# bleyerj/dolfinx_materials

Hardware: AMD Instinct MI355X
Metric: M quadrature-point updates/s (stress+tangent, fp64) (higher is better)
Workload: dtype f64; 1 GPU; cfg2: J2 von-Mises plasticity, linear isotropic hardening, small strain, 1e+07 Gauss points per GPU, stress + 6x6 consistent tangent, load/unload history increments 2-4; points_per_gpu=10000000, law=j2_linear, layout=AoS (N,6)/(N,36) boundary arrays in HBM, SoA resident state, placement=every array where its first allocation put it, settle_launches_before_warmup=560

## Files before the change

### dolfinx_materials_amd/csrc/dxmat.hip

```cpp
#include <hip/hip_runtime.h>

#include <algorithm>
#include <atomic>
#include <chrono>
#include <cmath>
#include <condition_variable>
#include <deque>
#include <map>
#include <mutex>
#include <thread>
#include <cstdarg>
#include <cstdio>
#include <cstdlib>
#include <cstring>
#include <string>
#include <vector>

#include "../../include/dxmat.h"
#include "dxm_common.hpp"
#include "fefp.hpp"
#include "gradient.hpp"
#include "small_strain.hpp"
#include "ramberg_osgood.hpp"
#include "param_fields.hpp"
#include "hyperelastic.hpp"
#include "hosford.hpp"
#include "orthotropic.hpp"
#include "host_side.hpp"

using namespace dxm;
static_assert(TL_FULL == DXM_TANGENT_FULL && TL_SYM == DXM_TANGENT_SYM && TL_COEF == DXM_TANGENT_COEF && TL_PACK4 == DXM_TANGENT_PACK4, "kernel and ABI layout ids");

static thread_local std::string g_last_error;

static int fail(int code, const char* fmt, ...) {
  char buf[512];
  va_list ap;
  va_start(ap, fmt);
  vsnprintf(buf, sizeof(buf), fmt, ap);
  va_end(ap);
  g_last_error = buf;
  return code;
}

#define HIP_TRY(expr)                                                                      \
  do {                                                                                     \
    hipError_t _e = (expr);                                                                \
    if (_e != hipSuccess) {                                                                \
      (void)hipGetLastError();                                                             \
      return fail(-2, "%s failed: %s (%s:%d)", #expr, hipGetErrorString(_e), __FILE__, __LINE__); \
    }                                                                                      \
  } while (0)

struct DeviceGuard {
  int prev = -1;
  bool ok = true;
  explicit DeviceGuard(int device) {
    if (hipGetDevice(&prev) != hipSuccess) prev = -1;
    if (prev != device) ok = (hipSetDevice(device) == hipSuccess);
  }
  ~DeviceGuard() {
    int cur = -1;
    if (prev >= 0 && hipGetDevice(&cur) == hipSuccess && cur != prev) (void)hipSetDevice(prev);
  }
};
#define DEVICE_GUARD(m)                                                        \
  DeviceGuard _guard((m)->device);                                             \
  if (!_guard.ok) return fail(-2, "hipSetDevice(%d) failed", (m)->device)

#ifdef DXM_CUSTOM_HARDENING
constexpr bool kCustomBuild = true;
#define DXM_STOCK_ONLY(entry) nullptr
#else
constexpr bool kCustomBuild = false;
#define DXM_STOCK_ONLY(entry) entry
#endif

struct dxm_material;

struct LaunchArgs {
  dxm_material* m;
  int grid;
  hipStream_t st;
  int64_t off, cnt;
  const double* grad;
  double* flux;
  double* ct;
  int stats_off;
  const MeshSource* fused;
  int tl;
};

constexpr unsigned L_FULL = 1u << TL_FULL, L_SYM = 1u << TL_SYM, L_COEF = 1u << TL_COEF, L_PACK4 = 1u << TL_PACK4;
constexpr unsigned L_ALL = L_FULL | L_SYM | L_COEF | L_PACK4;

struct LawDesc {
  int id;
  int n_grad, n_flux;
  int n_params, n_params_custom;
  int n_isv_fields;
  int n_fields;
  int isv_dim[DXM_MAX_STATE_FIELDS];
  const char* isv_name[DXM_MAX_STATE_FIELDS];
  int isv_slot[DXM_MAX_STATE_FIELDS];
  int n_slots;
  unsigned unit_fields;
  int alg_bytes;
  const char* kernel;
  const char* field_kernel;
  const char* no_fields;
  int (*build)(const double* p, LawParams& q);
  const char* stock_only;
  const void* (*residency_kernel)();
  int blocks_per_cu;
  unsigned set_layouts;
  const char* set_refusal;
  unsigned launch_layouts;
  const char* launch_refusal;
  const char* no_fused;
  const char* no_frame;
  const char* frame_kernel[2];
  void (*launch)(const LaunchArgs& a);
};

static int elastic_constants(const double* p, LawParams& q) {
  const double E = p[0], nu = p[1];
  if (!(E > 0.0) || !(nu > -1.0 && nu < 0.5)) return fail(-1, "invalid elastic constants E=%g nu=%g", E, nu);
  q.lambda = E * nu / (1 + nu) / (1 - 2 * nu);
  q.mu = E / 2 / (1 + nu);
  q.kappa = q.lambda + 2.0 * q.mu / 3.0;
  q.sig0 = 1.0;
  return 0;
}

static void yield_tolerance(LawParams& q) { q.tol = q.rtol * fmax(fabs(q.sig0), 2e-8 * q.mu); }

static int build_elastic(const double* p, LawParams& q) {
  if (int rc = elastic_constants(p, q)) return rc;
// ... 103 lines not shown
static void launch_hosford(const LaunchArgs& a);
static void launch_orthotropic(const LaunchArgs& a);

[[maybe_unused]] static const void* const kKernelOrder[5] = {
    (const void*)small_strain_kernel<LAW_ELASTIC, TL_FULL>, (const void*)small_strain_kernel<LAW_J2_LINEAR, TL_FULL>,
    (const void*)small_strain_kernel<LAW_J2_VOCE, TL_FULL>, (const void*)fefp_kernel<0, 0>, (const void*)fefp_kernel<1, 0>};


constexpr const char* kNoFrame = "this law is isotropic: a material frame changes nothing in its update, and accepting one would hide a "
                                 "mistake of the caller (frames are read by DXM_LAW_ORTHOTROPIC_ELASTIC)";

constexpr void state_field(LawDesc& d, int f, const char* name, int dim, int slot) {
  d.isv_name[f] = name; d.isv_dim[f] = dim; d.isv_slot[f] = slot;
}

constexpr LawDesc small_strain_law(int id, int n_params, int alg_bytes, const char* kernel, bool coef, void (*launch)(const LaunchArgs&)) {
  LawDesc d{};
  d.id = id;
  d.n_grad = d.n_flux = 6;
  d.n_params = d.n_params_custom = n_params;
  d.alg_bytes = alg_bytes;
  d.kernel = kernel;
  d.set_layouts = d.launch_layouts = coef ? L_ALL : L_FULL | L_SYM;
  d.no_frame = kNoFrame;
  d.launch = launch;
  return d;
}

constexpr void j2_state(LawDesc& d) {
  d.n_isv_fields = d.n_fields = 2;
  state_field(d, 0, "p", 1, 0);
  state_field(d, 1, "epsp", 6, 1);
  d.n_slots = SS_NSLOTS;
}

constexpr LawDesc law_elastic() {
  LawDesc d = small_strain_law(DXM_LAW_ELASTIC_ISO, 2, 384, "small_strain_kernel<0", false, launch_small_strain<LAW_ELASTIC>);
  d.build = build_elastic;
  d.residency_kernel = []() -> const void* { return (const void*)small_strain_kernel<LAW_ELASTIC, TL_FULL>; };
  d.blocks_per_cu = 32;
  d.set_refusal = d.launch_refusal = "the elastic tangent is the constant lambda 1x1 + 2 mu I: there are no per-point coefficients";
  d.no_fields = "the elastic tangent is a constant the host path never downloads";
  return d;
}

constexpr LawDesc law_j2_linear() {
  LawDesc d = small_strain_law(DXM_LAW_J2_LINEAR, 4, 496, "small_strain_kernel<1", true, launch_small_strain<LAW_J2_LINEAR>);
  j2_state(d);
  d.build = build_linear_hardening;
  d.residency_kernel = []() -> const void* { return (const void*)small_strain_kernel<LAW_J2_LINEAR, TL_FULL>; };
  d.blocks_per_cu = 32;
  d.field_kernel = "small_strain_field_kernel<1";
  return d;
}

constexpr LawDesc law_j2_voce() {
  LawDesc d = small_strain_law(DXM_LAW_J2_VOCE, 5, 496, "small_strain_kernel<2", true, launch_small_strain<LAW_J2_VOCE>);
  j2_state(d);
  d.n_params_custom = 9;
  d.build = build_voce_hardening;
  d.residency_kernel = []() -> const void* { return (const void*)small_strain_kernel<LAW_J2_VOCE, TL_FULL>; };
  d.blocks_per_cu = 256;
  d.field_kernel = "small_strain_field_kernel<2";
  return d;
}

// ... 135 lines not shown
static int tangent_size(const dxm_material* m);

static int isv_total(const LawDesc& d) {
  int t = 0;
  for (int f = 0; f < d.n_isv_fields; ++f) t += d.isv_dim[f];
  return t;
}

using dxm_host::HostPool;
using dxm_host::expand_coef_tangent;
using dxm_host::expand_pack4_tangent;
using dxm_host::expand_fefp_tangent;
using dxm_host::fill_const_tangent;
using dxm_host::CtRoute;
using dxm_host::Route;
static_assert(dxm_host::THIRD == SS_THIRD && dxm_host::FEFP_RECORD == FEFP_REC, "host rebuilds and kernels share these constants");

constexpr int DXM_MAX_CHUNKS = dxm_host::MAX_CHUNKS;
constexpr int DXM_RING = dxm_host::RING;

struct dxm_material {
  int law = 0;
  int device = 0;
  int64_t n = 0;
  int64_t ld = 0;
  LawParams prm{};
  std::vector<double> raw_params;
  int maxit = 25;
  double rtol = 1e-14;
  double* state[2] = {nullptr, nullptr};
  double* state_base = nullptr;
  size_t s1_skew = 0;
  bool s1_alias = false;
  BlockStats* d_stats = nullptr;
  BlockStats* h_stats = nullptr;
  int stats_capacity = 0;
  int last_grid = 0;
  hipStream_t pipe_stream = nullptr;
  hipStream_t down_stream2 = nullptr;
  hipEvent_t last_event = nullptr;
  bool last_event_recorded = false;
  bool launched = false;
  hipStream_t own_stream = nullptr;
  uint64_t epoch = 0;
  int parity = 0;
  bool opt_pipeline = true;
  bool opt_split_streams = true;
  int opt_packed_transfer = 2;
  bool opt_fused_gradient = true;
  bool opt_staged_gradient = true;
  bool opt_verbose = false;
  dxm_host::UploadChooser up;
  int last_upload = DXM_UPLOAD_NONE;
  int opt_host_threads = 16;
  int opt_pageable_dma = 0;
  int64_t opt_packed_min_points = 32768;
  int opt_max_chunks = DXM_MAX_CHUNKS;
  HostPool* pool = nullptr;
  double* h_coef = nullptr;
  int h_coef_per_point = 0;
  double* h_flux = nullptr;
  double* h_isv = nullptr;
  double elastic_lm[2] = {0.0, 0.0};
  hipEvent_t chunk_done[DXM_MAX_CHUNKS] = {};
  hipEvent_t kernel_done[DXM_MAX_CHUNKS] = {};
  int num_cu = 256;
  int blocks_per_cu = 5;
  int tangent_layout = 0;
  double* d_grad = nullptr;
  double* d_flux = nullptr;
  double* d_grad0 = nullptr;
  double* d_flux0 = nullptr;
  int io1_valid = 0;
  int io0_valid = 0;
  int opt_keep_initial_io = 0;
  double* d_isv = nullptr;
  double* isv_out[DXM_MAX_STATE_FIELDS] = {};
  double* d_isv_fields = nullptr;
  double* d_ct = nullptr;
  double* d_field = nullptr;
  double* h_grad_ring = nullptr;
  int64_t ring_slot_doubles = 0;
  hipEvent_t ring_done[DXM_RING] = {};
  int opt_stage_ahead = 3;
  double unregister_ms = 0.0;
  int pf_mask = 0;
  double* pf_law[2] = {nullptr, nullptr};
  double* pf_stream[PF_COUNT] = {};
  int frame_kind = 0;
  Frame9 frame_uniform{};
  double* frame_streams = nullptr;
};

static int sync_last(dxm_material* m);
static int pf_refresh_elastic(dxm_material* m, hipStream_t st);

static void free_state(dxm_material* m) {
  if (!m->state_base) return;
  (void)hipFree(m->state_base);
  m->state_base = nullptr;
}

static int build_params(dxm_material* m, const double* p, int np) {
  const LawDesc& d = kLaws[m->law];
  const int expect = n_params_of(d);
  if (np != expect) return fail(-1, "law %d expects %d parameters, got %d", m->law, expect, np);
  LawParams q{};
  q.maxit = m->maxit;
  q.rtol = m->rtol;
  if (int rc = d.build(p, q)) return rc;
  m->prm = q;
  m->raw_params.assign(p, p + np);
  return 0;
}

static int tangent_size(const dxm_material* m) {
  const LawDesc& d = kLaws[m->law];
  if (m->tangent_layout == DXM_TANGENT_SYM) return d.n_flux * (d.n_flux + 1) / 2;
  if (m->tangent_layout == DXM_TANGENT_COEF) return 9;
  if (m->tangent_layout == DXM_TANGENT_PACK4) return 4;
  return d.n_flux * d.n_grad;
}

__global__ void fill_slot_kernel(double* dst, int64_t count, double value) {
  const int64_t i = (int64_t)blockIdx.x * blockDim.x + threadIdx.x;
  if (i < count) dst[i] = value;
}

struct PackMap { int n; int slot[16]; };

__global__ void __launch_bounds__(256) ring_upload_kernel(const double2_t* __restrict__ src, double2_t* __restrict__ dst, int64_t n16) {
  for (int64_t k = (int64_t)blockIdx.x * blockDim.x + threadIdx.x; k < n16; k += (int64_t)gridDim.x * blockDim.x)
    dst[k] = __builtin_nontemporal_load(src + k);
// ... 36 lines not shown

int dxm_law_info_get(int law, dxm_law_info* out) {
  if (!law_known(law) || !out) return fail(-1, "unknown law id %d", law);
  const LawDesc& d = kLaws[law];
  memset(out, 0, sizeof(*out));
  out->n_grad = d.n_grad;
  out->n_flux = d.n_flux;
  out->n_params = n_params_of(d);
  out->n_isv_fields = d.n_isv_fields;
  for (int f = 0; f < DXM_MAX_STATE_FIELDS; ++f) {
    out->isv_dim[f] = d.isv_dim[f];
    out->isv_name[f] = d.isv_name[f];
  }
  out->n_isv_total = isv_total(d);
  out->algorithmic_bytes_per_point = d.alg_bytes;
  return 0;
}

static int init_state(dxm_material* m) {
  const LawDesc& d = kLaws[m->law];
  if (d.n_slots == 0) return 0;
  const size_t bytes = (size_t)d.n_slots * m->ld * sizeof(double);
  for (int w = 0; w < 2; ++w) {
    HIP_TRY(hipMemsetAsync(m->state[w], 0, bytes, m->own_stream));
    for (int f = 0; f < d.n_fields; ++f) {
      if (!(d.unit_fields & (1u << f))) continue;
      for (int s = d.isv_slot[f]; s < d.isv_slot[f] + 3; ++s) {
        const int blocks = (int)((m->ld + 255) / 256);
        hipLaunchKernelGGL(fill_slot_kernel, dim3(blocks), dim3(256), 0, m->own_stream,
                           m->state[w] + (size_t)s * m->ld, m->ld, 1.0);
      }
    }
  }
  HIP_TRY(hipStreamSynchronize(m->own_stream));
  return 0;
}

dxm_material* dxm_create(int law, const double* params, int n_params, int64_t npoints, int device) {
  if (!law_known(law)) { fail(-1, "unknown law id %d", law); return nullptr; }
  if (npoints < 0) { fail(-1, "negative point count"); return nullptr; }
  int ndev = 0;
  hipError_t e = hipGetDeviceCount(&ndev);
  if (e != hipSuccess || ndev <= 0) {
    fail(-2, "no usable HIP device (hipGetDeviceCount: %s, count %d); libdxmat has no CPU fallback",
         hipGetErrorString(e), ndev);
    return nullptr;
  }
  if (device < 0 || device >= ndev) { fail(-1, "device %d out of range [0,%d)", device, ndev); return nullptr; }
  const LawDesc& d = kLaws[law];
  if (kCustomBuild && d.stock_only) { fail(-1, "%s", d.stock_only); return nullptr; }
  dxm_material* m = new dxm_material();
  m->law = law;
  m->device = device;
  m->n = npoints;
  m->ld = ((npoints + 255) / 256) * 256 + 32;
  auto bail = [&](void) -> dxm_material* { dxm_destroy(m); return nullptr; };
  if (build_params(m, params, n_params) != 0) return bail();
  DeviceGuard guard(device);
  if (!guard.ok) { fail(-2, "hipSetDevice(%d) failed", device); return bail(); }
  hipDeviceProp_t prop;
  if (hipGetDeviceProperties(&prop, device) == hipSuccess) m->num_cu = prop.multiProcessorCount;
  if (hipStreamCreateWithFlags(&m->own_stream, hipStreamNonBlocking) != hipSuccess ||
      hipEventCreateWithFlags(&m->last_event, hipEventDisableTiming) != hipSuccess) {
    fail(-2, "hipStreamCreate / hipEventCreate failed"); return bail();
  }
  if (d.n_slots > 0) {
    const size_t bytes = (size_t)d.n_slots * m->ld * sizeof(double);
    {
      if (hipMalloc(&m->state_base, 2 * bytes + m->s1_skew) != hipSuccess) {
        fail(-3, "hipMalloc of %zu state bytes failed", 2 * bytes + m->s1_skew); return bail();
      }
      m->state[0] = m->state_base;
      m->state[1] = reinterpret_cast<double*>(reinterpret_cast<char*>(m->state_base) + bytes + m->s1_skew);
    }
  }
  {
    hipFuncAttributes fa;
    if (d.residency_kernel && hipFuncGetAttributes(&fa, d.residency_kernel()) == hipSuccess && fa.numRegs > 0) {
      const int alloc = ((fa.numRegs + 7) / 8) * 8;
      int waves_simd = 512 / alloc;
      if (waves_simd > 8) waves_simd = 8;
      int by_vgpr = waves_simd * 4 / WAVES_PER_BLOCK;
      int by_lds = fa.sharedSizeBytes > 0 ? (int)(160 * 1024 / fa.sharedSizeBytes) : 8;
      int occ = by_vgpr < by_lds ? by_vgpr : by_lds;
      if (occ < 1) occ = 1;
      m->blocks_per_cu = occ;
    }
    if (d.blocks_per_cu) m->blocks_per_cu = d.blocks_per_cu;
  }
  m->stats_capacity = dxm_host::stats_capacity(m->num_cu, npoints);
  if (hipMalloc(&m->d_stats, sizeof(BlockStats) * m->stats_capacity) != hipSuccess) {
    fail(-3, "hipMalloc of stats failed"); return bail();
  }
  if (init_state(m) != 0) return bail();
  g_last_error.clear();
  return m;
}

int dxm_destroy(dxm_material* m) {
  if (!m) return 0;
  DeviceGuard guard(m->device);
  (void)sync_last(m);
  delete m->pool;
  if (m->h_coef) (void)hipHostFree(m->h_coef);
  if (m->h_flux) (void)hipHostFree(m->h_flux);
  if (m->h_isv) (void)hipHostFree(m->h_isv);
// ... 174 lines not shown
  }
  int devi = 0;
  if (int rc = current_device_index(&devi)) return rc;
  std::lock_guard<std::mutex> lk(g_staging_mu[devi]);
  Staging* s = nullptr;
  if (int rc = staging_for_current_device(&s)) return rc;
  const size_t nchunks = (bytes + BOUNCE_BYTES - 1) / BOUNCE_BYTES;
  for (size_t c = 0; c < nchunks; ++c) {
    if (c >= 2) HIP_TRY(hipEventSynchronize(s->done[c & 1]));
    memcpy(s->buf + (c & 1) * BOUNCE_BYTES, static_cast<const char*>(host) + c * BOUNCE_BYTES, chunk_size(c, nchunks, bytes));
    HIP_TRY(hipMemcpyAsync(static_cast<char*>(dev) + c * BOUNCE_BYTES, s->buf + (c & 1) * BOUNCE_BYTES, chunk_size(c, nchunks, bytes),
                           hipMemcpyHostToDevice, st));
    HIP_TRY(hipEventRecord(s->done[c & 1], st));
  }
  HIP_TRY(hipStreamSynchronize(st));
  return 0;
}

int dxm_set_state(dxm_material* m, int which, int field, const double* host_aos) {
  if (int rc = check_field(m, which, field)) return rc;
  if (!host_aos) return fail(-1, "null host pointer");
  DEVICE_GUARD(m);
  if (int rc = sync_last(m)) return rc;
  const LawDesc& d = kLaws[m->law];
  const int dim = d.isv_dim[field];
  const int64_t n = m->n;
  if (n == 0) return 0;
  if (int rc = materialize_s1(m)) return rc;
  if (!m->d_field) HIP_TRY(hipMalloc(&m->d_field, sizeof(double) * n * 6));
  PackMap map{};
  map.n = dim;
  for (int c = 0; c < dim; ++c) map.slot[c] = d.isv_slot[field] + c;
  hipStream_t st = m->own_stream;
  if (int rc = upload_from_host(m->d_field, host_aos, sizeof(double) * n * dim, st)) return rc;
  const int blocks = (int)((n * dim + 255) / 256);
  hipLaunchKernelGGL(unpack_isv_kernel, dim3(blocks), dim3(256), 0, st, state_of(m, which), m->ld, n,
                     m->d_field, map);
  HIP_TRY(hipGetLastError());
  HIP_TRY(hipStreamSynchronize(st));
  return 0;
}

int dxm_get_state(dxm_material* m, int which, int field, double* host_aos) {
  if (int rc = check_field(m, which, field)) return rc;
  if (!host_aos) return fail(-1, "null host pointer");
  DEVICE_GUARD(m);
  if (int rc = sync_last(m)) return rc;
  const LawDesc& d = kLaws[m->law];
  const int dim = d.isv_dim[field];
  const int64_t n = m->n;
  if (n == 0) return 0;
  if (!m->d_field) HIP_TRY(hipMalloc(&m->d_field, sizeof(double) * n * 6));
  PackMap map{};
  map.n = dim;
  for (int c = 0; c < dim; ++c) map.slot[c] = d.isv_slot[field] + c;
  hipStream_t st = m->own_stream;
  const int blocks = (int)((n * dim + 255) / 256);
  hipLaunchKernelGGL(pack_isv_kernel, dim3(blocks), dim3(256), 0, st, state_of(m, which), m->ld, n,
                     m->d_field, map);
  HIP_TRY(hipGetLastError());
  return download_to_host(host_aos, m->d_field, sizeof(double) * n * dim, st);
}

int dxm_advance(dxm_material* m) {
  if (!m) return fail(-1, "null handle");
  if (!m->s1_alias) {
// ... 25 lines not shown
  if (kind != 0 && kind != 1) return fail(-1, "kind must be 0 (gradient) or 1 (flux)");
  if (!(io_mask(m, which) & (1 << kind)))
    return fail(-1, "the %s of that state is not held on the device (a host-buffer integrate; for s0 also option keep_initial_io before dxm_advance)", kind ? "flux" : "gradient");
  if (m->n == 0) return 0;
  if (!host_aos) return fail(-1, "null host pointer");
  DEVICE_GUARD(m);
  if (int rc = sync_last(m)) return rc;
  const LawDesc& d = kLaws[m->law];
  const bool first = which == DXM_S0 || m->s1_alias;
  const double* src = kind ? (first ? m->d_flux0 : m->d_flux) : (first ? m->d_grad0 : m->d_grad);
  return download_to_host(host_aos, src, sizeof(double) * m->n * (kind ? d.n_flux : d.n_grad), m->own_stream);
}

int dxm_revert(dxm_material* m) {
  if (!m) return fail(-1, "null handle");
  m->s1_alias = true;
  m->io1_valid = 0;
  return 0;
}

}

template <int LAW>
static void launch_small_strain(const LaunchArgs& a) {
  dxm_material* m = a.m;
  const int grid = a.grid, tl = a.tl;
  const hipStream_t st = a.st;
  const int64_t cnt = a.cnt;
  const double* grad = a.grad;
  double *flux = a.flux, *ct = a.ct;
  const double* s0 = m->state[0] + a.off;
  double* s1 = m->state[1] + a.off;
  BlockStats* bs = m->d_stats + a.stats_off;
  const MeshSource none{};
  const MeshSource& src = a.fused ? *a.fused : none;
  const int g = a.fused ? a.fused->kind : 0;
  constexpr int dyn_lds = LAW == LAW_ELASTIC ? 0 : 2304;
#ifndef DXM_CUSTOM_HARDENING
  if constexpr (LAW != LAW_ELASTIC) {
    if (m->pf_mask) {
      ParamStreams pf{};
      for (int k = 0; k < PF_COUNT; ++k) pf.p[k] = m->pf_stream[k] ? m->pf_stream[k] + a.off : nullptr;
      param_fields_launch(LAW, tl, g, grid, dyn_lds, st, m->prm, pf, cnt, grad, s0, s1, m->ld, flux, ct, bs, src);
      return;
    }
  }
#endif
#define DXM_LAUNCH_SS(TL, G)                                                                              \
  hipLaunchKernelGGL((small_strain_kernel<LAW, TL, G>), dim3(grid), dim3(BLOCK), dyn_lds, st, m->prm, cnt, grad, s0, s1, \
                     m->ld, flux, ct, bs, src)
#define DXM_LAUNCH_SS_G(TL) do { if (g == 0) DXM_LAUNCH_SS(TL, 0); else if (g == 1) DXM_LAUNCH_SS(TL, 1); \
                                 else if (g == 2) DXM_LAUNCH_SS(TL, 2); else DXM_LAUNCH_SS(TL, 3); } while (0)
  if (tl == TL_SYM) DXM_LAUNCH_SS_G(TL_SYM);
  else if (tl == TL_FULL) DXM_LAUNCH_SS_G(TL_FULL);
  else if constexpr (ss_has_coef<LAW>) { if (tl == TL_PACK4) DXM_LAUNCH_SS_G(TL_PACK4); else DXM_LAUNCH_SS_G(TL_COEF); }
#undef DXM_LAUNCH_SS_G
#undef DXM_LAUNCH_SS
}

static void launch_fefp(const LaunchArgs& a, bool voce) {
  dxm_material* m = a.m;
  const int grid = a.grid;
  const hipStream_t st = a.st;
  const int64_t cnt = a.cnt;
  const double* grad = a.grad;
  double *flux = a.flux, *ct = a.ct;
  const double* s0 = m->state[0] + a.off;
  double* s1 = m->state[1] + a.off;
  BlockStats* bs = m->d_stats + a.stats_off;
  const MeshSource none{};
  const MeshSource& fsrc = a.fused ? *a.fused : none;
  const int g = a.fused ? a.fused->kind : 0;
#define DXM_LAUNCH_FEFP(HARD, G, T) \
  hipLaunchKernelGGL((fefp_kernel<HARD, G, T>), dim3(grid), dim3(BLOCK), 0, st, m->prm, cnt, grad, s0, s1, m->ld, flux, ct, bs, fsrc)
#define DXM_LAUNCH_FEFP_G(HARD, T) do { if (g == 0) DXM_LAUNCH_FEFP(HARD, 0, T); else if (g == 1) DXM_LAUNCH_FEFP(HARD, 1, T); \
                                       else if (g == 2) DXM_LAUNCH_FEFP(HARD, 2, T); else DXM_LAUNCH_FEFP(HARD, 3, T); } while (0)
  if (a.tl == TL_COEF) { if (voce) DXM_LAUNCH_FEFP_G(1, 1); else DXM_LAUNCH_FEFP_G(0, 1); }
  else                 { if (voce) DXM_LAUNCH_FEFP_G(1, 0); else DXM_LAUNCH_FEFP_G(0, 0); }
#undef DXM_LAUNCH_FEFP_G
#undef DXM_LAUNCH_FEFP
}
static void launch_fefp_voce(const LaunchArgs& a) { launch_fefp(a, true); }
static void launch_fefp_linear(const LaunchArgs& a) { launch_fefp(a, false); }

#ifndef DXM_CUSTOM_HARDENING
static void launch_ramberg_osgood(const LaunchArgs& a) {
  const MeshSource none{};
  ramberg_osgood_launch(a.tl, a.fused ? a.fused->kind : 0, a.grid, a.st, a.m->prm, a.cnt, a.grad, a.flux, a.ct,
                        a.m->d_stats + a.stats_off, a.fused ? *a.fused : none);
}

static void launch_ogden(const LaunchArgs& a) {
  dxm_material* m = a.m;
  ogden_launch(a.grid, a.st, m->prm, a.cnt, a.grad, m->state[1] + a.off, m->ld, a.flux, a.ct, m->d_stats + a.stats_off);
}

static void launch_hosford(const LaunchArgs& a) {
  dxm_material* m = a.m;
  hosford_launch(a.tl, a.grid, a.st, m->prm, a.cnt, a.grad, m->state[0] + a.off, m->state[1] + a.off, m->ld, a.flux, a.ct,
                 m->d_stats + a.stats_off);
}

static void launch_orthotropic(const LaunchArgs& a) {
  dxm_material* m = a.m;
  orthotropic_launch(m->frame_kind, a.tl, a.grid, a.st, m->prm, a.cnt, a.grad, m->frame_uniform,
                     m->frame_streams ? m->frame_streams + a.off : nullptr, m->ld, a.flux, a.ct, m->d_stats + a.stats_off);
}
#endif

static int launch_range(dxm_material* m, int64_t off, int64_t cnt, const double* grad, double* flux,
                        double* ct, hipStream_t st, int stats_off, int* grid_out,
                        const MeshSource* fused, int tl) {
  if (((uintptr_t)grad | (uintptr_t)flux | (uintptr_t)ct) & 15)
    return fail(-1, "gradient / flux / tangent device arrays must be 16-byte aligned");
  m->io1_valid = 0;
  static_assert(WAVE * WAVES_PER_BLOCK == 256, "dxm_host::launch_grid counts workgroups of 256 points");
  const int64_t blocks = dxm_host::launch_grid(cnt, m->num_cu, m->blocks_per_cu);
  if (stats_off + blocks > m->stats_capacity) return fail(-1, "internal: stats buffer too small");
  const int grid = (int)blocks;
  const LawDesc& d = kLaws[m->law];
  if (!d.launch) return fail(-1, "law %d not launchable", m->law);
  if (fused && d.no_fused) return fail(-1, "%s", d.no_fused);
  if (!(d.launch_layouts & (1u << tl))) return fail(-1, "%s", d.launch_refusal);
  d.launch(LaunchArgs{m, grid, st, off, cnt, grad, flux, ct, stats_off, fused, tl});
  HIP_TRY(hipGetLastError());
  *grid_out = grid;
  return 0;
}

static int launch(dxm_material* m, const double* grad, double* flux, double* ct, hipStream_t st,
                  const MeshSource* fused = nullptr) {
  if (m->n == 0) { m->last_grid = 0; return 0; }
  int grid = 0;
  if (int rc = launch_range(m, 0, m->n, grad, flux, ct, st, 0, &grid, fused, m->tangent_layout)) return rc;
  m->last_grid = grid;
  m->launched = true;
  m->s1_alias = false;
  hipStreamCaptureStatus cap = hipStreamCaptureStatusNone;
  if (hipStreamIsCapturing(st, &cap) != hipSuccess) { (void)hipGetLastError(); cap = hipStreamCaptureStatusNone; }
  m->last_event_recorded = false;
  if (cap == hipStreamCaptureStatusNone) {
    HIP_TRY(hipEventRecord(m->last_event, st));
    m->last_event_recorded = true;
  }
  return 0;
}

extern "C" {

int dxm_integrate_device(dxm_material* m, const double* grad_dev, double dt, double* flux_dev,
                         double* ct_dev, void* hip_stream) {
  (void)dt;
  if (!m) return fail(-1, "null handle");
  if (m->n > 0 && (!grad_dev || !flux_dev || !ct_dev)) return fail(-1, "null device pointer");
  DEVICE_GUARD(m);
  return launch(m, grad_dev, flux_dev, ct_dev, (hipStream_t)hip_stream);
}
// ... 650 lines not shown

int dxm_integrate_displacement_rows(dxm_material* m, dxm_mesh* mesh, const double* u_host, double dt, double* flux_rows,
                                    double* ct_rows, const int64_t* rows, dxm_stats* stats) {
  (void)dt;
  if (!m) return fail(-1, "null argument");
  if (m->n > 0 && (!flux_rows || !ct_rows || !rows)) return fail(-1, "dxm_integrate_displacement_rows needs the flux array, the tangent array and the row index");
  return integrate_displacement_host(m, mesh, u_host, flux_rows, nullptr, ct_rows, stats, rows);
}

int dxm_integrate_displacement_device(dxm_material* m, dxm_mesh* mesh, const double* u_dev, double dt,
                                      double* flux_dev, double* ct_dev, void* hip_stream) {
  (void)dt;
  if (!m || !mesh) return fail(-1, "null argument");
  if (mesh->device != m->device) return fail(-1, "mesh and material live on different devices");
  if (dxm_mesh_npoints(mesh) != m->n) return fail(-1, "mesh has %lld Gauss points, material %lld",
                                                   (long long)dxm_mesh_npoints(mesh), (long long)m->n);
  if (m->n > 0 && (!u_dev || !flux_dev || !ct_dev)) return fail(-1, "null device pointer");
  DEVICE_GUARD(m);
  hipStream_t st = (hipStream_t)hip_stream;
  const LawDesc& d = kLaws[m->law];
  if (m->opt_fused_gradient && fusable(mesh)) {
    const MeshSource src = mesh_source(mesh, u_dev);
    return launch(m, flux_dev , flux_dev, ct_dev, st, &src);
  }
  if (!m->d_grad) HIP_TRY(hipMalloc(&m->d_grad, sizeof(double) * m->n * d.n_grad));
  if (int rc = dxm_mesh_gradient_device(mesh, u_dev, gradient_kind(d), m->d_grad, hip_stream)) return rc;
  return launch(m, m->d_grad, flux_dev, ct_dev, st);
}

const double* dxm_state_ptr(const dxm_material* m, int which, int field, int comp) {
  if (check_field(m, which, field)) return nullptr;
  const LawDesc& d = kLaws[m->law];
  if (comp < 0 || comp >= d.isv_dim[field]) { fail(-1, "component out of range"); return nullptr; }
  return state_of(m, which) + (size_t)(d.isv_slot[field] + comp) * m->ld;
}

const char* dxm_kernel_name(const dxm_material* m) {
  if (!m) return "";
  if (m->frame_kind) return kLaws[m->law].frame_kernel[m->frame_kind - 1];
  return m->pf_mask ? kLaws[m->law].field_kernel : kLaws[m->law].kernel;
}

int dxm_expand_tangent_device(const double* coef_dev, int64_t npoints, double* ct_dev, int device, void* hip_stream) {
  if (npoints < 0) return fail(-1, "negative point count");
  if (npoints == 0) return 0;
  if (!coef_dev || !ct_dev) return fail(-1, "null device pointer");
  if (((uintptr_t)coef_dev | (uintptr_t)ct_dev) & 15) return fail(-1, "coefficient / tangent device arrays must be 16-byte aligned");
  DeviceGuard guard(device);
  if (!guard.ok) return fail(-2, "hipSetDevice(%d) failed", device);
  const int64_t tiles = (npoints + WAVE - 1) / WAVE;
  int64_t blocks = (tiles + WAVES_PER_BLOCK - 1) / WAVES_PER_BLOCK;
  if (blocks > 256 * 32) blocks = 256 * 32;
  hipLaunchKernelGGL(expand_tangent_kernel, dim3((unsigned)blocks), dim3(BLOCK), 0, (hipStream_t)hip_stream, npoints, coef_dev, ct_dev);
  HIP_TRY(hipGetLastError());
  return 0;
}

int dxm_expand_tangent_pack4_device(const double* flux_dev, const double* pack_dev, int64_t npoints, double* ct_dev, int device,
                                    void* hip_stream) {
  if (npoints < 0) return fail(-1, "negative point count");
  if (npoints == 0) return 0;
  if (!flux_dev || !pack_dev || !ct_dev) return fail(-1, "null device pointer");
  if (((uintptr_t)flux_dev | (uintptr_t)pack_dev | (uintptr_t)ct_dev) & 15) return fail(-1, "stress / pack / tangent device arrays must be 16-byte aligned");
  DeviceGuard guard(device);
  if (!guard.ok) return fail(-2, "hipSetDevice(%d) failed", device);
  const int64_t tiles = (npoints + WAVE - 1) / WAVE;
// ... 243 lines not shown
int dxm_set_option(dxm_material* m, const char* name, double value) {
  if (!m || !name) return fail(-1, "null argument");
  const std::string k(name);
  const bool on = value != 0.0;
  if (k == "pipeline") m->opt_pipeline = on;
  else if (k == "split_streams") m->opt_split_streams = on;
  else if (k == "packed_transfer") {
    if (!(value == 0.0 || value == 1.0 || value == 2.0)) return fail(-1, "packed_transfer must be 0, 1 or 2");
    m->opt_packed_transfer = (int)value;
  }
  else if (k == "fused_gradient") m->opt_fused_gradient = on;
  else if (k == "verbose") m->opt_verbose = on;
  else if (k == "stage_ahead") {
    if (!(value >= 1 && value <= DXM_RING - 2)) return fail(-1, "stage_ahead must be in [1, %d]", DXM_RING - 2);
    m->opt_stage_ahead = (int)value;
  }
  else if (k == "register_input") {
    if (!(value == 0.0 || value == 1.0 || value == 2.0)) return fail(-1, "register_input must be 0, 1 or 2");
    m->up.set_option((int)value);
  }
  else if (k == "keep_initial_io") m->opt_keep_initial_io = on;
  else if (k == "pageable_dma") m->opt_pageable_dma = value != 0.0;
  else if (k == "query_foreign_pointers") g_query_foreign.store(on ? 1 : 0);
  else if (k == "packed_min_points") {
    if (!(value >= 0 && value <= 1e12)) return fail(-1, "packed_min_points must be >= 0");
    m->opt_packed_min_points = (int64_t)value;
  }
  else if (k == "host_threads") {
    if (!(value >= 1 && value <= 256)) return fail(-1, "host_threads must be in [1, 256]");
    m->opt_host_threads = (int)value;
  } else if (k == "max_chunks") {
    if (!(value >= 1 && value <= DXM_MAX_CHUNKS)) return fail(-1, "max_chunks must be in [1, %d]", DXM_MAX_CHUNKS);
    m->opt_max_chunks = (int)value;
  } else if (k == "blocks_per_cu") {
    if (!(value >= 1 && value <= 256)) return fail(-1, "blocks_per_cu must be in [1, 256]");
    m->blocks_per_cu = (int)value;
  } else {
    return fail(-1, "unknown option '%s'", name);
  }
  ++m->epoch;
  return 0;
}

int dxm_isv_host(dxm_material* m, int which, double* isv_aos) {
  if (!m) return fail(-1, "null handle");
  if (which != DXM_S0 && which != DXM_S1) return fail(-1, "state selector must be DXM_S0 or DXM_S1");
  const LawDesc& d = kLaws[m->law];
  const int total = isv_total(d);
  if (total == 0 || m->n == 0) return 0;
  if (!isv_aos) return fail(-1, "null host pointer");
  DEVICE_GUARD(m);
  if (int rc = sync_last(m)) return rc;
  if (!m->d_isv) HIP_TRY(hipMalloc(&m->d_isv, sizeof(double) * m->n * total));
  if (int rc = pack_isv_range(m, which, 0, m->n, m->d_isv, m->own_stream)) return rc;
  return download_to_host(isv_aos, m->d_isv, sizeof(double) * m->n * total, m->own_stream);
}

int dxm_host_copy(void* dst, const void* src, uint64_t bytes, int threads) {
  if (bytes == 0) return 0;
  if (!dst || !src) return fail(-1, "null host pointer");
  dxm_host::host_copy(dst, src, bytes, threads);
  return 0;
}

static int move_rows(bool scatter, double* dst, const double* src, const int64_t* rows, int64_t n, int width, int threads) {
  if (n <= 0 || width <= 0) return 0;
// ... 41 lines not shown
```

### dolfinx_materials_amd/csrc/small_strain_body.hpp

```cpp
  __shared__ __attribute__((aligned(16))) double lds_all[WAVES_PER_BLOCK * SS_LDS_PER_WAVE];
  __shared__ unsigned long long red[4 * WAVES_PER_BLOCK];

  int lane = threadIdx.x & (WAVE - 1);
  const int wid = threadIdx.x >> 6;
  double* stage = lds_all + wid * SS_LDS_PER_WAVE;
  double* coef = stage + SS_STAGE;
  double2_t* stage2 = reinterpret_cast<double2_t*>(stage);

  const int64_t ntiles = (n + WAVE - 1) / WAVE;
  const int64_t tile_stride = (int64_t)gridDim.x * WAVES_PER_BLOCK;

  unsigned long long c_plastic = 0, c_notconv = 0, c_nan = 0, c_maxit = 0;

  const double lambda_u = prm.lambda, mu_u = prm.mu;

  for (int64_t tile = (int64_t)blockIdx.x * WAVES_PER_BLOCK + wid; tile < ntiles;
       tile += tile_stride) {
    const int64_t base = tile * WAVE;
    const int npts = (n - base) < WAVE ? (int)(n - base) : WAVE;
    if constexpr (FIELDS || LAW == LAW_J2_VOCE || LAW == LAW_RAMBERG_OSGOOD) {
      asm volatile("" : "+v"(lane));
      lane &= WAVE - 1;
    }
    const bool valid = lane < npts;
    const int64_t gi = base + lane;

    double e[6];
    double p_n = 0.0, ep[6] = {0, 0, 0, 0, 0, 0};
    if constexpr (GRAD == 0) {
#include "tile_rows6_load.hpp"
      if constexpr (ss_has_state<LAW>) {
        if (valid) {
          p_n = stream_load<3>(s0 + gi);
#pragma unroll
          for (int c = 0; c < 6; ++c) ep[c] = stream_load<3>(s0 + (int64_t)(1 + c) * ld + gi);
        }
      }
      wave_lds_sync();
#include "tile_rows6_take.hpp"
      wave_lds_sync();
    } else {
      double Hd[9];
      if constexpr (GRAD == 1) {
        {
          const int64_t cell = ((src.point0 + base) >> 3) + (lane >> 3);
          double2_t r0 = {0.0, 0.0}, r1 = {0.0, 0.0}, r2 = {0.0, 0.0};
          if (cell < src.ncells) {
            const int64_t nd = src.conn[cell * 8 + (lane & 7)];
            r0 = double2_t{src.coords[3 * nd], src.coords[3 * nd + 1]};
            r1 = double2_t{src.coords[3 * nd + 2], src.u[3 * nd]};
            r2 = double2_t{src.u[3 * nd + 1], src.u[3 * nd + 2]};
          }
          double2_t* d = reinterpret_cast<double2_t*>(coef + (lane >> 3) * HEX_FUSED_REC + (lane & 7) * 6);
          d[0] = r0; d[1] = r1; d[2] = r2;
        }
        wave_lds_sync();
        {
          const double2_t* rec = reinterpret_cast<const double2_t*>(coef + (lane >> 3) * HEX_FUSED_REC);
          auto node = [&](int m, double* X, double* U) {
            const double2_t a = rec[m * 3], b = rec[m * 3 + 1], c = rec[m * 3 + 2];
            X[0] = a.x; X[1] = a.y; X[2] = b.x;
            U[0] = b.y; U[1] = c.x; U[2] = c.y;
          };
          const int q = lane & 7;
          if (valid) {
            hex8_disp_grad(src.xi[q][0], src.xi[q][1], src.xi[q][2], node, Hd);
          } else {
#pragma unroll
            for (int k = 0; k < 9; ++k) Hd[k] = 0.0;
          }
        }
        wave_lds_sync();
      } else {
        if (valid) {
          const int64_t cell = (src.point0 + gi) / src.nqp;
          if constexpr (GRAD == 2) tet4_cell_disp_grad(src.coords, src.conn, src.u, cell, Hd);
          else simplex_disp_grad(src, cell, (int)(src.point0 + gi - cell * src.nqp), Hd);
        } else {
#pragma unroll
          for (int k = 0; k < 9; ++k) Hd[k] = 0.0;
        }
      }
      {
        const double r = 0.70710678118654752440;
        e[0] = Hd[0]; e[1] = Hd[4]; e[2] = Hd[8];
        e[3] = r * (Hd[1] + Hd[3]); e[4] = r * (Hd[2] + Hd[6]); e[5] = r * (Hd[5] + Hd[7]);
      }
      if constexpr (ss_has_state<LAW>) {
        if (valid) {
          p_n = stream_load<3>(s0 + gi);
#pragma unroll
          for (int c = 0; c < 6; ++c) ep[c] = stream_load<3>(s0 + (int64_t)(1 + c) * ld + gi);
        }
      }
    }

    double lambda = lambda_u, mu = mu_u;
    LawParams lp_point;
    const LawParams& lp = FIELDS ? lp_point : prm;
    if constexpr (FIELDS) {
      lp_point = prm;
      if (pf.p[PF_LAMBDA] && valid) lambda = stream_load<3>(pf.p[PF_LAMBDA] + gi);
      if (pf.p[PF_MU] && valid) mu = stream_load<3>(pf.p[PF_MU] + gi);
      if (pf.p[PF_SIG0] && valid) lp_point.sig0 = stream_load<3>(pf.p[PF_SIG0] + gi);
      if (pf.p[PF_H1] && valid) lp_point.h1 = stream_load<3>(pf.p[PF_H1] + gi);
      if constexpr (LAW == LAW_J2_VOCE) {
        if (pf.p[PF_H2] && valid) lp_point.h2 = stream_load<3>(pf.p[PF_H2] + gi);
        if (pf.p[PF_SIG0] || pf.p[PF_MU]) lp_point.tol = prm.rtol * fmax(fabs(lp.sig0), 2e-8 * mu);
      }
    }
    double c1 = lambda, c2 = 2.0 * mu, c3 = 0.0;
    double wn = 0.0;
    double p_new = p_n;
    if constexpr (ss_has_state<LAW>) {
#pragma unroll
      for (int c = 0; c < 6; ++c) e[c] -= ep[c];
      const double tr = e[0] + e[1] + e[2];
      const double third = tr / 3.0;
      double se[6];
      se[0] = 2.0 * mu * (e[0] - third);
      se[1] = 2.0 * mu * (e[1] - third);
      se[2] = 2.0 * mu * (e[2] - third);
      se[3] = 2.0 * mu * e[3];
      se[4] = 2.0 * mu * e[4];
      se[5] = 2.0 * mu * e[5];
      double nrm2 = 0.0;
#pragma unroll
      for (int c = 0; c < 6; ++c) nrm2 += se[c] * se[c];
      const double seq = sqrt(1.5 * nrm2);
      const double f = seq - hardening_R<LAW>(lp, p_n);
      if (f > 0.0) {
        double dp;
        unsigned iters = 0;
        if constexpr (LAW == LAW_J2_LINEAR) {
          dp = f / (lp.h1 + 3.0 * mu);
        } else {
          dp = 0.0;
          const double tolp = fmax(lp.tol, prm.rtol * seq);
          for (int it = 0;; ++it) {
            const double r = seq - 3.0 * mu * dp - hardening_R<LAW>(lp, p_n + dp);
            if (fabs(r) <= tolp) break;
            if (it >= prm.maxit) { if (valid) ++c_notconv; break; }
            const double dr = -3.0 * mu - hardening_dR<LAW>(lp, p_n + dp);
            dp -= r / dr;
            ++iters;
          }
        }
        const double iseq = 1.0 / seq;
        double nn[6];
#pragma unroll
        for (int c = 0; c < 6; ++c) nn[c] = 1.5 * se[c] * iseq;
        const double beta = dp * iseq;
        {
          const double rho = 1.0 - 3.0 * mu * beta;
          wn = rho > 0.0 ? 1.5 * iseq / rho : 0.0;
          if constexpr (LAW != LAW_J2_LINEAR) { if (valid && !(rho > 0.0)) ++c_notconv; }
          else if ((FIELDS && pf.p[PF_H1]) ? lp.h1 < 0.0 : prm.h1 < 0.0) { if (valid && !(rho > 0.0)) ++c_notconv; }
        }
        const double gamma = 1.0 / (hardening_dR<LAW>(lp, p_n + dp) + 3.0 * mu);
        c1 = lambda + 2.0 * mu * mu * beta;
        c2 = 2.0 * mu - 6.0 * mu * mu * beta;
        c3 = 4.0 * mu * mu * (beta - gamma);
        p_new = p_n + dp;
#pragma unroll
        for (int c = 0; c < 6; ++c) {
          ep[c] += dp * nn[c];
          e[c] -= dp * nn[c];
        }
        if (valid) {
          ++c_plastic;
          c_maxit = iters > c_maxit ? iters : c_maxit;
        }
      }
    }
    const double ltr = lambda * (e[0] + e[1] + e[2]);
    double s[6];
    if constexpr (LAW == LAW_RAMBERG_OSGOOD) {
      ramberg_osgood_update(prm, mu, e, stage2 + lane * 3, s, c1, c2, c3, wn, valid, c_plastic, c_notconv, c_maxit);
    } else {
    s[0] = ltr + 2.0 * mu * e[0];
    s[1] = ltr + 2.0 * mu * e[1];
    s[2] = ltr + 2.0 * mu * e[2];
    s[3] = 2.0 * mu * e[3];
    s[4] = 2.0 * mu * e[4];
    s[5] = 2.0 * mu * e[5];
    }
    {
      const double chk = s[0] + s[1] + s[2] + s[3] + s[4] + s[5] + p_new + ((c1 + c2) + (c3 + wn));
      if (valid && !(fabs(chk) <= 1.79769313486231570e308)) ++c_nan;
    }

    if constexpr (ss_has_state<LAW>) {
      if (valid) {
        stream_store<1>(s1 + gi, p_new);
#pragma unroll
        for (int c = 0; c < 6; ++c) stream_store<1>(s1 + (int64_t)(1 + c) * ld + gi, ep[c]);
      }
    }

    stage2[lane * 3 + 0] = double2_t{s[0], s[1]};
    stage2[lane * 3 + 1] = double2_t{s[2], s[3]};
    stage2[lane * 3 + 2] = double2_t{s[4], s[5]};
    if constexpr (ss_has_coef<LAW> && TL == TL_PACK4) {
      double2_t* c4 = reinterpret_cast<double2_t*>(coef) + lane * 2;
      c4[0] = double2_t{c1, c2};
      c4[1] = double2_t{c3, wn};
    } else if constexpr (ss_has_coef<LAW>) {
#include "small_strain_stage_coef.hpp"
    }
    wave_lds_sync();

#include "tile_rows6_store.hpp"
    if constexpr (TL == TL_PACK4) {
      static_assert(ss_has_coef<LAW>, "the elastic tangent is a constant: nothing to write");
      if (npts == WAVE) {
        double2_t* gct = reinterpret_cast<double2_t*>(ct + base * 4);
        const double2_t* c4 = reinterpret_cast<const double2_t*>(coef);
        stream_store<0>(gct + lane, c4[lane]);
        stream_store<0>(gct + WAVE + lane, c4[WAVE + lane]);
      } else {
        double2_t* gct = reinterpret_cast<double2_t*>(ct + base * 4);
        const double2_t* c4 = reinterpret_cast<const double2_t*>(coef);
        if (lane < npts * 2) stream_store<0>(gct + lane, c4[lane]);
        if (WAVE + lane < npts * 2) stream_store<0>(gct + WAVE + lane, c4[WAVE + lane]);
      }
    } else if constexpr (TL == TL_COEF) {
      static_assert(ss_has_coef<LAW>, "the elastic tangent is a constant: nothing to write");
      if (npts == WAVE) {
        double2_t* gct = reinterpret_cast<double2_t*>(ct + base * 9);
        const double2_t* c2 = reinterpret_cast<const double2_t*>(coef);
// ... 89 lines not shown
```

Baseline: 10720 Mpoints/s.

## Skip state writeback for wave tiles whose state stayed unchanged

Adds a per-wave byte flag array recording whether a tile's two state buffers already hold identical values. In the J2 kernels, a wave skips its seven state stores when no valid lane yielded and the flag says the output buffer already matches, then updates the flag. This removes a large share of HBM write traffic for elastic points during load/unload history. In exchange it adds flag bookkeeping: host memsets when the state is exposed, edited or captured, a separate kernel instantiation, and a ballot plus a flag load per wave.

```diff
diff --git a/dolfinx_materials_amd/csrc/dxmat.hip b/dolfinx_materials_amd/csrc/dxmat.hip
--- a/dolfinx_materials_amd/csrc/dxmat.hip
+++ b/dolfinx_materials_amd/csrc/dxmat.hip
@@ -23,6 +23,7 @@
 #include "small_strain.hpp"
 #include "ramberg_osgood.hpp"
 #include "param_fields.hpp"
+#include "state_skip.hpp"
 #include "hyperelastic.hpp"
 #include "hosford.hpp"
 #include "orthotropic.hpp"
@@ -89,6 +90,7 @@
   int stats_off;
   const MeshSource* fused;
   int tl;
+  unsigned char* tile_same;
 };
 
 constexpr unsigned L_FULL = 1u << TL_FULL, L_SYM = 1u << TL_SYM, L_COEF = 1u << TL_COEF, L_PACK4 = 1u << TL_PACK4;
@@ -104,6 +106,7 @@
   const char* isv_name[DXM_MAX_STATE_FIELDS];
   int isv_slot[DXM_MAX_STATE_FIELDS];
   int n_slots;
+  bool tile_flags;
   unsigned unit_fields;
   int alg_bytes;
   const char* kernel;
@@ -273,6 +276,7 @@
   state_field(d, 0, "p", 1, 0);
   state_field(d, 1, "epsp", 6, 1);
   d.n_slots = SS_NSLOTS;
+  d.tile_flags = !kCustomBuild;
 }
 
 constexpr LawDesc law_elastic() {
@@ -474,6 +478,11 @@
   double* state_base = nullptr;
   size_t s1_skew = 0;
   bool s1_alias = false;
+  unsigned char* tile_same = nullptr;
+  bool tile_same_zero = false;
+  bool launch_refused = false;
+  bool exposed = false;
+  bool opt_skip_unchanged = true;
   BlockStats* d_stats = nullptr;
   BlockStats* h_stats = nullptr;
   int stats_capacity = 0;
@@ -538,9 +547,20 @@
 static int pf_refresh_elastic(dxm_material* m, hipStream_t st);
 
 static void free_state(dxm_material* m) {
+  if (m->tile_same) (void)hipFree(m->tile_same);
+  m->tile_same = nullptr;
   if (!m->state_base) return;
   (void)hipFree(m->state_base);
   m->state_base = nullptr;
+}
+
+static size_t tile_flag_bytes(const dxm_material* m) { return (size_t)((m->ld + WAVE - 1) / WAVE); }
+
+static int zero_tile_flags(dxm_material* m) {
+  if (!m->tile_same) return 0;
+  HIP_TRY(hipMemsetAsync(m->tile_same, 0, tile_flag_bytes(m), m->own_stream));
+  m->tile_same_zero = true;
+  return 0;
 }
 
 static int build_params(dxm_material* m, const double* p, int np) {
@@ -643,6 +663,7 @@
       }
     }
   }
+  if (m->tile_same) HIP_TRY(hipMemsetAsync(m->tile_same, 1, tile_flag_bytes(m), m->own_stream));
   HIP_TRY(hipStreamSynchronize(m->own_stream));
   return 0;
 }
@@ -683,6 +704,9 @@
       }
       m->state[0] = m->state_base;
       m->state[1] = reinterpret_cast<double*>(reinterpret_cast<char*>(m->state_base) + bytes + m->s1_skew);
+    }
+    if (d.tile_flags && hipMalloc(&m->tile_same, tile_flag_bytes(m)) != hipSuccess) {
+      fail(-3, "hipMalloc of %zu tile flag bytes failed", tile_flag_bytes(m)); return bail();
     }
   }
   {
@@ -923,6 +947,7 @@
   map.n = dim;
   for (int c = 0; c < dim; ++c) map.slot[c] = d.isv_slot[field] + c;
   hipStream_t st = m->own_stream;
+  if (int rc = zero_tile_flags(m)) return rc;
   if (int rc = upload_from_host(m->d_field, host_aos, sizeof(double) * n * dim, st)) return rc;
   const int blocks = (int)((n * dim + 255) / 256);
   hipLaunchKernelGGL(unpack_isv_kernel, dim3(blocks), dim3(256), 0, st, state_of(m, which), m->ld, n,
@@ -1014,6 +1039,7 @@
   const double* s0 = m->state[0] + a.off;
   double* s1 = m->state[1] + a.off;
   BlockStats* bs = m->d_stats + a.stats_off;
+  unsigned char* const same = a.tile_same;
   const MeshSource none{};
   const MeshSource& src = a.fused ? *a.fused : none;
   const int g = a.fused ? a.fused->kind : 0;
@@ -1023,7 +1049,12 @@
     if (m->pf_mask) {
       ParamStreams pf{};
       for (int k = 0; k < PF_COUNT; ++k) pf.p[k] = m->pf_stream[k] ? m->pf_stream[k] + a.off : nullptr;
-      param_fields_launch(LAW, tl, g, grid, dyn_lds, st, m->prm, pf, cnt, grad, s0, s1, m->ld, flux, ct, bs, src);
+      if (same) m->launch_refused = !state_skip_launch(LAW, tl, g, grid, dyn_lds, st, m->prm, &pf, cnt, grad, s0, s1, m->ld, flux, ct, bs, src, same);
+      else param_fields_launch(LAW, tl, g, grid, dyn_lds, st, m->prm, pf, cnt, grad, s0, s1, m->ld, flux, ct, bs, src);
+      return;
+    }
+    if (same) {
+      m->launch_refused = !state_skip_launch(LAW, tl, g, grid, dyn_lds, st, m->prm, nullptr, cnt, grad, s0, s1, m->ld, flux, ct, bs, src, same);
       return;
     }
   }
@@ -1090,6 +1121,14 @@
 }
 #endif
 
+static bool flagged_kernel_exists(const dxm_material* m, int tl, const MeshSource* fused) {
+#ifdef DXM_CUSTOM_HARDENING
+  return false;
+#else
+  return state_skip_serves(m->law, m->pf_mask != 0, tl, fused ? fused->kind : 0);
+#endif
+}
+
 static int launch_range(dxm_material* m, int64_t off, int64_t cnt, const double* grad, double* flux,
                         double* ct, hipStream_t st, int stats_off, int* grid_out,
                         const MeshSource* fused, int tl) {
@@ -1104,7 +1143,24 @@
   if (!d.launch) return fail(-1, "law %d not launchable", m->law);
   if (fused && d.no_fused) return fail(-1, "%s", d.no_fused);
   if (!(d.launch_layouts & (1u << tl))) return fail(-1, "%s", d.launch_refusal);
-  d.launch(LaunchArgs{m, grid, st, off, cnt, grad, flux, ct, stats_off, fused, tl});
+  unsigned char* same = nullptr;
+  if (m->tile_same) {
+    if (m->opt_skip_unchanged && !m->exposed && off % WAVE == 0 && flagged_kernel_exists(m, tl, fused)) {
+      same = m->tile_same + off / WAVE;
+      m->tile_same_zero = false;
+    } else {
+      hipStreamCaptureStatus cap = hipStreamCaptureStatusNone;
+      if (hipStreamIsCapturing(st, &cap) != hipSuccess) { (void)hipGetLastError(); cap = hipStreamCaptureStatusActive; }
+      const bool capturing = cap != hipStreamCaptureStatusNone;
+      if (capturing || !m->tile_same_zero) {
+        HIP_TRY(hipMemsetAsync(m->tile_same, 0, tile_flag_bytes(m), st));
+        if (!capturing) m->tile_same_zero = true;
+      }
+    }
+  }
+  m->launch_refused = false;
+  d.launch(LaunchArgs{m, grid, st, off, cnt, grad, flux, ct, stats_off, fused, tl, same});
+  if (m->launch_refused) return fail(-1, "internal: no kernel with tile flags for this form of law %d (state_skip_serves said there was)", m->law);
   HIP_TRY(hipGetLastError());
   *grid_out = grid;
   return 0;
@@ -1821,6 +1877,11 @@
   if (check_field(m, which, field)) return nullptr;
   const LawDesc& d = kLaws[m->law];
   if (comp < 0 || comp >= d.isv_dim[field]) { fail(-1, "component out of range"); return nullptr; }
+  if (m->tile_same && !m->exposed) {
+    dxm_material* w = const_cast<dxm_material*>(m);
+    w->exposed = true;
+    ++w->epoch;
+  }
   return state_of(m, which) + (size_t)(d.isv_slot[field] + comp) * m->ld;
 }
 
@@ -2130,6 +2191,14 @@
   } else if (k == "max_chunks") {
     if (!(value >= 1 && value <= DXM_MAX_CHUNKS)) return fail(-1, "max_chunks must be in [1, %d]", DXM_MAX_CHUNKS);
     m->opt_max_chunks = (int)value;
+  } else if (k == "skip_unchanged_state") {
+    if (on && !m->opt_skip_unchanged && m->tile_same) {
+      DEVICE_GUARD(m);
+      if (int rc = sync_last(m)) return rc;
+      if (int rc = zero_tile_flags(m)) return rc;
+      HIP_TRY(hipStreamSynchronize(m->own_stream));
+    }
+    m->opt_skip_unchanged = on;
   } else if (k == "blocks_per_cu") {
     if (!(value >= 1 && value <= 256)) return fail(-1, "blocks_per_cu must be in [1, 256]");
     m->blocks_per_cu = (int)value;
diff --git a/dolfinx_materials_amd/csrc/small_strain_body.hpp b/dolfinx_materials_amd/csrc/small_strain_body.hpp
--- a/dolfinx_materials_amd/csrc/small_strain_body.hpp
+++ b/dolfinx_materials_amd/csrc/small_strain_body.hpp
@@ -27,6 +27,11 @@
 
     double e[6];
     double p_n = 0.0, ep[6] = {0, 0, 0, 0, 0, 0};
+#ifdef DXM_TILE_FLAGS
+    constexpr bool FLAG_LATE = FIELDS && LAW == LAW_J2_VOCE;
+    unsigned same = 0;
+    bool yielded = false;
+#endif
     if constexpr (GRAD == 0) {
 #include "tile_rows6_load.hpp"
       if constexpr (ss_has_state<LAW>) {
@@ -35,6 +40,9 @@
 #pragma unroll
           for (int c = 0; c < 6; ++c) ep[c] = stream_load<3>(s0 + (int64_t)(1 + c) * ld + gi);
         }
+#ifdef DXM_TILE_FLAGS
+        if constexpr (!FLAG_LATE) same = tile_same[tile];
+#endif
       }
       wave_lds_sync();
 #include "tile_rows6_take.hpp"
@@ -92,6 +100,9 @@
 #pragma unroll
           for (int c = 0; c < 6; ++c) ep[c] = stream_load<3>(s0 + (int64_t)(1 + c) * ld + gi);
         }
+#ifdef DXM_TILE_FLAGS
+        if constexpr (!FLAG_LATE) same = tile_same[tile];
+#endif
       }
     }
 
@@ -130,6 +141,9 @@
       const double seq = sqrt(1.5 * nrm2);
       const double f = seq - hardening_R<LAW>(lp, p_n);
       if (f > 0.0) {
+#ifdef DXM_TILE_FLAGS
+        yielded = true;
+#endif
         double dp;
         unsigned iters = 0;
         if constexpr (LAW == LAW_J2_LINEAR) {
@@ -191,11 +205,21 @@
     }
 
     if constexpr (ss_has_state<LAW>) {
+#ifdef DXM_TILE_FLAGS
+      if constexpr (FLAG_LATE) same = tile_same[tile];
+      const bool changed = __builtin_amdgcn_ballot_w64(valid && yielded) != 0;
+      if (changed || __builtin_amdgcn_readfirstlane(same) != 1u) {
+#endif
       if (valid) {
         stream_store<1>(s1 + gi, p_new);
 #pragma unroll
         for (int c = 0; c < 6; ++c) stream_store<1>(s1 + (int64_t)(1 + c) * ld + gi, ep[c]);
       }
+#ifdef DXM_TILE_FLAGS
+        const unsigned now = changed ? 0u : 1u;
+        if (lane == 0 && same != now) tile_same[tile] = (unsigned char)now;
+      }
+#endif
     }
 
     stage2[lane * 3 + 0] = double2_t{s[0], s[1]};
diff --git a/dolfinx_materials_amd/csrc/state_skip.hip b/dolfinx_materials_amd/csrc/state_skip.hip
--- /dev/null
+++ b/dolfinx_materials_amd/csrc/state_skip.hip
@@ -0,0 +1,76 @@
+#include "state_skip.hpp"
+
+#define DXM_UPDATE_KERNELS_ONLY
+#include "small_strain.hpp"
+
+namespace dxm {
+namespace skip {
+
+#define DXM_TILE_FLAGS
+template <int LAW, int TL, int GRAD = 0>
+__global__ void __launch_bounds__(BLOCK, 4)
+small_strain_kernel(const LawParams prm, const int64_t n, const double* __restrict__ eps,
+                    const double* __restrict__ s0, double* __restrict__ s1, const int64_t ld,
+                    double* __restrict__ sig, double* __restrict__ ct,
+                    BlockStats* __restrict__ stats, const MeshSource src, unsigned char* __restrict__ tile_same) {
+  static_assert(ss_has_state<LAW>, "tile flags: the laws with state");
+  constexpr bool FIELDS = false;
+  constexpr ParamStreams pf = {};
+#include "small_strain_body.hpp"
+}
+
+template <int LAW, int TL, int GRAD = 0>
+__global__ void __launch_bounds__(BLOCK, 4)
+small_strain_field_kernel(const LawParams prm, const ParamStreams pf, const int64_t n, const double* __restrict__ eps,
+                          const double* __restrict__ s0, double* __restrict__ s1, const int64_t ld,
+                          double* __restrict__ sig, double* __restrict__ ct,
+                          BlockStats* __restrict__ stats, const MeshSource src, unsigned char* __restrict__ tile_same) {
+  static_assert(ss_has_state<LAW>, "tile flags: the laws with state");
+  constexpr bool FIELDS = true;
+#include "small_strain_body.hpp"
+}
+#undef DXM_TILE_FLAGS
+
+constexpr bool serves(int law, bool fields, int tl, int grad_kind) {
+  return !(law == LAW_J2_VOCE && fields && tl == TL_SYM && grad_kind == 3);
+}
+
+template <int LAW>
+static void launch(int tl, int g, int grid, int dyn_lds, hipStream_t st, const LawParams& prm, const ParamStreams* pf, int64_t cnt,
+                   const double* grad, const double* s0, double* s1, int64_t ld, double* flux, double* ct, BlockStats* bs,
+                   const MeshSource& src, unsigned char* tile_same) {
+#define DXM_LAUNCH_SKIP(TL, G)                                                                                                    \
+  do {                                                                                                                            \
+    if (!pf) hipLaunchKernelGGL((small_strain_kernel<LAW, TL, G>), dim3(grid), dim3(BLOCK), dyn_lds, st, prm, cnt, grad, s0, s1, ld, \
+                                flux, ct, bs, src, tile_same);                                                                    \
+    else if constexpr (serves(LAW, true, TL, G))                                                                                  \
+      hipLaunchKernelGGL((small_strain_field_kernel<LAW, TL, G>), dim3(grid), dim3(BLOCK), dyn_lds, st, prm, *pf, cnt, grad, s0, s1, \
+                         ld, flux, ct, bs, src, tile_same);                                                                       \
+  } while (0)
+#define DXM_LAUNCH_SKIP_G(TL) do { if (g == 0) DXM_LAUNCH_SKIP(TL, 0); else if (g == 1) DXM_LAUNCH_SKIP(TL, 1); \
+                                   else if (g == 2) DXM_LAUNCH_SKIP(TL, 2); else DXM_LAUNCH_SKIP(TL, 3); } while (0)
+  if (tl == TL_SYM) DXM_LAUNCH_SKIP_G(TL_SYM);
+  else if (tl == TL_FULL) DXM_LAUNCH_SKIP_G(TL_FULL);
+  else if (tl == TL_PACK4) DXM_LAUNCH_SKIP_G(TL_PACK4);
+  else DXM_LAUNCH_SKIP_G(TL_COEF);
+#undef DXM_LAUNCH_SKIP_G
+#undef DXM_LAUNCH_SKIP
+}
+
+}
+
+bool state_skip_serves(int law, bool fields, int tl, int grad_kind) {
+  return (law == LAW_J2_LINEAR || law == LAW_J2_VOCE) && skip::serves(law, fields, tl, grad_kind);
+}
+
+bool state_skip_launch(int law, int tl, int grad_kind, int grid, int dyn_lds, hipStream_t st, const LawParams& prm, const ParamStreams* pf,
+                       int64_t cnt, const double* grad, const double* s0, double* s1, int64_t ld, double* flux, double* ct,
+                       BlockStats* bs, const MeshSource& src, unsigned char* tile_same) {
+  if (!state_skip_serves(law, pf != nullptr, tl, grad_kind)) return false;
+  if (law == LAW_J2_LINEAR) skip::launch<LAW_J2_LINEAR>(tl, grad_kind, grid, dyn_lds, st, prm, pf, cnt, grad, s0, s1, ld, flux, ct, bs, src, tile_same);
+  else if (law == LAW_J2_VOCE) skip::launch<LAW_J2_VOCE>(tl, grad_kind, grid, dyn_lds, st, prm, pf, cnt, grad, s0, s1, ld, flux, ct, bs, src, tile_same);
+  else return false;
+  return true;
+}
+
+}
diff --git a/dolfinx_materials_amd/csrc/state_skip.hpp b/dolfinx_materials_amd/csrc/state_skip.hpp
--- /dev/null
+++ b/dolfinx_materials_amd/csrc/state_skip.hpp
@@ -0,0 +1,18 @@
+#pragma once
+#include <hip/hip_runtime.h>
+
+#include "dxm_common.hpp"
+#include "gradient.hpp"
+#include "param_fields.hpp"
+
+namespace dxm {
+
+__attribute__((visibility("hidden"))) bool state_skip_serves(int law, bool fields, int tl, int grad_kind);
+
+__attribute__((visibility("hidden"))) bool state_skip_launch(int law, int tl, int grad_kind, int grid, int dyn_lds, hipStream_t st,
+                                                             const LawParams& prm, const ParamStreams* pf, int64_t cnt,
+                                                             const double* grad, const double* s0, double* s1, int64_t ld,
+                                                             double* flux, double* ct, BlockStats* bs, const MeshSource& src,
+                                                             unsigned char* tile_same);
+
+}
```

Measured after the change: 11100 Mpoints/s, median of 5. 1.04x the previous value.
